# Lukeasargen/Show-Attend-and-Tell-Pytorch-Lightning

Measured on AMD Instinct MI355X. Metric: captions/sec (train step) at B=128, 256px, seq_len=22, higher is better.
Workload: dtype bf16; 1 GPU; C2: resnet50 encoder_size=7 encoder_dim=512 vocab=6400 T=22, 128 images/GPU x R=5 captions, trainable encoder, Adam, full lengths, decoder_tf=always; global_batch_images=128, parallelism=dp1, grad_bucket_dtype=fp32

## Files before the change

### show-attend-and-tell-pytorch-lightning_amd/csrc/wgrad3x3.hip

```cpp
#include <stdlib.h>

#include "gemm_bf16_common.h"
#include "profile.h"

namespace sat {

typedef int i32x4 __attribute__((ext_vector_type(4)));
typedef __attribute__((address_space(3))) void* lptr3_t;
__device__ void raw_buffer_load_lds_w(i32x4 rsrc, lptr3_t lds, int size, int voffset, int soffset, int offset, int aux) __asm("llvm.amdgcn.raw.buffer.load.lds");

namespace {
constexpr int W3_OOB = (int)0x80000000;
constexpr int W3_WAVES = 9, W3_THREADS = 64 * W3_WAVES;
constexpr int W3_MAXP = 4;
constexpr int W3_STAGES = 3;

__device__ __forceinline__ i32x4 w3_rsrc(const void* base) {
    const unsigned long long b = reinterpret_cast<unsigned long long>(base);
    i32x4 r;
    r[0] = (int)(unsigned)b; r[1] = (int)(unsigned)((b >> 32) & 0xFFFF);
    r[2] = W3_OOB; r[3] = 0x00020000;
    return r;
}

struct W3Args {
    const __bf16* dy; const __bf16* x; float* out;
    int Nimg, H, W, C, K;
    int nr;
    int units;
    int per;
    int HP;
    int Z;
};

__global__ __launch_bounds__(W3_THREADS) void wgrad3x3_kernel(W3Args a) {
    extern __shared__ __attribute__((aligned(1024))) __bf16 smem[];
    const int tid = threadIdx.x, lane = tid & 63, wave = tid >> 6;
    const int ci0 = blockIdx.x * 64, co0 = blockIdx.y * 64, bz = blockIdx.z;
    const int W = a.W, H = a.H, C = a.C, K = a.K, nr = a.nr, HW2 = W + 2;
    const int STAGE = 64 * 64 + a.HP * 64;
    const int u0 = bz * a.per, u1 = min(a.units, u0 + a.per);
    const int upi = H / nr;
    const i32x4 rA = w3_rsrc(a.dy), rX = w3_rsrc(a.x);

    const int npieces = 8 + a.HP / 8;
    int p_off[W3_MAXP]; int p_hr[W3_MAXP]; bool p_dy[W3_MAXP], p_on[W3_MAXP], p_colok[W3_MAXP]; int p_lds[W3_MAXP];
#pragma unroll
    for (int j = 0; j < W3_MAXP; ++j) {
        const int piece = j * W3_WAVES + wave;
        p_on[j] = piece < npieces; p_dy[j] = piece < 8; p_hr[j] = 0; p_colok[j] = false; p_off[j] = 0;
        const int sl = lane & 7;
        if (p_dy[j]) {
            const int krow = piece * 8 + (lane >> 3);
            const int lq = (sl >> 2) ^ ((krow >> 1) & 1);
            p_off[j] = (krow * K + co0 + (lq * 4 + (sl & 3)) * 8) * 2;
            p_lds[j] = piece * 512;
        } else {
            const int hp = (piece - 8) * 8 + (lane >> 3);
            const int hr = hp / HW2, hc = hp - hr * HW2 - 1;
            const int lq = (sl >> 2) ^ ((hp >> 1) & 1);
            p_hr[j] = hr;
            p_colok[j] = p_on[j] && hr < nr + 2 && hc >= 0 && hc < W;
            p_off[j] = ((hr * W + hc) * C + ci0 + (lq * 4 + (sl & 3)) * 8) * 2;
            p_lds[j] = 64 * 64 + (piece - 8) * 512;
        }
    }
    auto issue = [&](int buf, int u) {
        const int n = u / upi, p0 = (u - n * upi) * nr;
        const int baseA = ((n * H + p0) * W) * K * 2;
        const int baseX = ((n * H + p0 - 1) * W) * C * 2;
        __bf16* st = smem + buf * STAGE;
#pragma unroll
        for (int j = 0; j < W3_MAXP; ++j) {
            if (!p_on[j]) continue;
            if (p_dy[j]) raw_buffer_load_lds_w(rA, (lptr3_t)(st + p_lds[j]), 16, p_off[j] + baseA, 0, 0, 0);
            else {
                const int ih = p0 - 1 + p_hr[j];
                const bool ok = p_colok[j] && ih >= 0 && ih < H;
                raw_buffer_load_lds_w(rX, (lptr3_t)(st + p_lds[j]), 16, ok ? p_off[j] + baseX : W3_OOB, 0, 0, 0);
            }
        }
    };

    const int tg = lane >> 4, ti = lane & 15;
    const int t_h = tg >> 1, t_mh = tg & 1, t_q = ti >> 2, t_p = ti & 3;
    const int tap_r = wave / 3, tap_s = wave - tap_r * 3;
    int a_off[2];
#pragma unroll
    for (int i = 0; i < 2; ++i) {
        const int col = i * 32 + 16 * t_mh + 4 * t_p, kr = 8 * t_h + t_q;
        a_off[i] = kr * 64 + (((col >> 5) ^ ((kr >> 1) & 1)) << 5) + (col & 31);
    }
    int b_off[4][2][2];
#pragma unroll
    for (int ks = 0; ks < 4; ++ks)
#pragma unroll
        for (int hf = 0; hf < 2; ++hf) {
            const int k = ks * 16 + 8 * t_h + t_q + 4 * hf;
            const int pr = k / W, q = k - pr * W;
            const int hp = (pr + tap_r) * HW2 + q + tap_s;
#pragma unroll
            for (int j = 0; j < 2; ++j) {
                const int col = j * 32 + 16 * t_mh + 4 * t_p;
                b_off[ks][hf][j] = 64 * 64 + hp * 64 + (((col >> 5) ^ ((hp >> 1) & 1)) << 5) + (col & 31);
            }
        }

    f32x16 acc[2][2];
#pragma unroll
    for (int i = 0; i < 2; ++i)
#pragma unroll
        for (int j = 0; j < 2; ++j)
#pragma unroll
            for (int r = 0; r < 16; ++r) acc[i][j][r] = 0.f;

    int mine = 0;
#pragma unroll
    for (int j = 0; j < W3_MAXP; ++j) mine += p_on[j] ? 1 : 0;
    mine = __builtin_amdgcn_readfirstlane(mine);
    if (u0 < u1) {
        issue(0, u0);
        if (u0 + 1 < u1) issue(1, u0 + 1);
        int cur = 0, nxt = 2;
        for (int u = u0; u < u1; ++u) {
            if (u + 1 < u1) {
                if (mine == 4) asm volatile("s_waitcnt vmcnt(4)" ::: "memory");
                else if (mine == 3) asm volatile("s_waitcnt vmcnt(3)" ::: "memory");
                else if (mine == 2) asm volatile("s_waitcnt vmcnt(2)" ::: "memory");
                else asm volatile("s_waitcnt vmcnt(0)" ::: "memory");
            } else asm volatile("s_waitcnt vmcnt(0)" ::: "memory");
            asm volatile("s_waitcnt lgkmcnt(0)" ::: "memory");
            __builtin_amdgcn_s_barrier();
            asm volatile("" ::: "memory");
            if (u + 2 < u1) issue(nxt, u + 2);
            const __bf16* st = smem + cur * STAGE;
#pragma unroll
            for (int ks = 0; ks < 4; ++ks) {
                bf16x8 af[2], bf[2];
#pragma unroll
                for (int i = 0; i < 2; ++i) {
                    const __bf16* p = st + a_off[i] + ks * 16 * 64;
                    bf16x4 lo = __builtin_amdgcn_ds_read_tr16_b64_v4bf16((__attribute__((address_space(3))) bf16x4*)p);
                    bf16x4 hi = __builtin_amdgcn_ds_read_tr16_b64_v4bf16((__attribute__((address_space(3))) bf16x4*)(p + 4 * 64));
                    af[i] = __builtin_shufflevector(lo, hi, 0, 1, 2, 3, 4, 5, 6, 7);
                }
#pragma unroll
                for (int j = 0; j < 2; ++j) {
                    bf16x4 lo = __builtin_amdgcn_ds_read_tr16_b64_v4bf16((__attribute__((address_space(3))) bf16x4*)(st + b_off[ks][0][j]));
                    bf16x4 hi = __builtin_amdgcn_ds_read_tr16_b64_v4bf16((__attribute__((address_space(3))) bf16x4*)(st + b_off[ks][1][j]));
                    bf[j] = __builtin_shufflevector(lo, hi, 0, 1, 2, 3, 4, 5, 6, 7);
                }
#pragma unroll
                for (int i = 0; i < 2; ++i)
#pragma unroll
                    for (int j = 0; j < 2; ++j) acc[i][j] = __builtin_amdgcn_mfma_f32_32x32x16_bf16(af[i], bf[j], acc[i][j], 0, 0, 0);
            }
            cur = (cur + 1 == W3_STAGES) ? 0 : cur + 1;
            nxt = (nxt + 1 == W3_STAGES) ? 0 : nxt + 1;
        }
    }
    const int li = lane & 31, lh = lane >> 5;
    const long N9 = 9L * C;
    float* out = a.out + (a.Z > 1 ? (long)bz * K * N9 : 0L);
#pragma unroll
    for (int i = 0; i < 2; ++i)
#pragma unroll
        for (int j = 0; j < 2; ++j)
#pragma unroll
            for (int r = 0; r < 16; ++r) {
                const int row = co0 + i * 32 + (r & 3) + 8 * (r >> 2) + 4 * lh;
                const int col = ci0 + j * 32 + li;
                out[(long)row * N9 + (long)wave * C + col] = acc[i][j][r];
            }
}
}

int wgrad3x3_eligible(const ConvGeom& g) {
    if (!dev_switch(SW_WGRAD3X3)) return 0;
    if (g.R != 3 || g.S != 3 || g.stride != 1 || g.pad != 1 || (g.sw && g.sw != 1)) return 0;
    if (g.C % 64 || g.K % 64) return 0;
    if (g.H != g.P || g.W != g.Q) return 0;
    if (!(g.W == 8 || g.W == 16 || g.W == 32 || g.W == 64)) return 0;
    if (g.H % (64 / g.W)) return 0;
    if ((long)g.N * g.H * g.W * (g.C > g.K ? g.C : g.K) >= (1L << 30)) return 0;
    return 1;
}

int launch_wgrad3x3(const void* dy, const void* x, float* dw, const ConvGeom& g, float* slab, long slab_elems, hipStream_t st) {
    W3Args a;
    a.dy = reinterpret_cast<const __bf16*>(dy); a.x = reinterpret_cast<const __bf16*>(x);
    a.Nimg = g.N; a.H = g.H; a.W = g.W; a.C = g.C; a.K = g.K;
    a.nr = 64 / g.W; a.units = g.N * (g.H / a.nr);
    a.HP = ((a.nr + 2) * (g.W + 2) + 7) / 8 * 8;
    SAT_REQUIRE(8 + a.HP / 8 <= W3_WAVES * W3_MAXP, "wgrad3x3: %d LDS-DMA pieces per k-tile", 8 + a.HP / 8);
    const long tiles = (long)(g.C / 64) * (g.K / 64), out_elems = (long)g.K * 9 * g.C;
    static const int target = getenv("SAT_W3_TARGET") ? atoi(getenv("SAT_W3_TARGET")) : 256;
    long z = target / tiles; if (z < 1) z = 1;
    if (z > a.units / 8) z = a.units / 8 > 0 ? a.units / 8 : 1;
    while (z > 1 && (!slab || z * out_elems > slab_elems)) --z;
    a.per = (int)cdiv(a.units, z); a.Z = (int)cdiv(a.units, a.per);
    a.out = a.Z > 1 ? slab : dw;
    const size_t lds = W3_STAGES * (size_t)(64 * 64 + a.HP * 64) * sizeof(__bf16);
    static bool attr_set = false;
    if (!attr_set) {
        SAT_CHECK_HIP(hipFuncSetAttribute(reinterpret_cast<const void*>(&wgrad3x3_kernel), hipFuncAttributeMaxDynamicSharedMemorySize, 128 * 1024));
        attr_set = true;
    }
    {
        char pname[128];
        if (profile_enabled()) {
            static const bool shapes = getenv("SAT_PROFILE_SHAPES") != nullptr;
            if (shapes) snprintf(pname, sizeof pname, "gemm_wgrad3x3 M%d N%d K%d z%d", g.K, 9 * g.C, g.N * g.H * g.W, a.Z);
            else snprintf(pname, sizeof pname, "gemm_wgrad3x3");
        }
        ProfScope prof(pname, 2.0 * g.K * 9.0 * g.C * g.N * g.H * g.W, 2.0 * g.N * g.H * g.W * ((double)g.C + g.K) + 4.0 * out_elems, st);
        hipLaunchKernelGGL(wgrad3x3_kernel, dim3(g.C / 64, g.K / 64, a.Z), dim3(W3_THREADS), lds, st, a);
        SAT_TRY(launch_ok("wgrad3x3_kernel"));
        if (a.Z > 1) {
            BArgs k{};
            k.M = g.K; k.N = 9 * g.C; k.C = dw; k.ldc = 9 * g.C; k.slab = slab; k.nsplit = a.Z; k.wide_store = 1; k.wide_slab = 1; k.epi = EPI_NONE;
            SAT_TRY(launch_splitk_reduce<float>(k, st));
        }
    }
    return SAT_OK;
}

}
```

Measured before the change: 32510 captions/s.

## Restructure 3x3 wgrad kernel with row-ring input reuse and deeper pipeline

Rewrites the 3x3 weight-gradient kernel to keep input rows in an LDS ring buffer, so consecutive row units reuse the overlapping halo rows and load only the new rows. Waves go from 9 to 12, each owning one filter row tap and a 32x32 quadrant with three accumulators. The k-tile pipeline is deeper, with loads issued between k-steps and waits computed from outstanding counts. The kernel is templated on width, uses inline-asm buffer-to-LDS loads, and adds optional timestamp instrumentation. In exchange it needs more LDS (up to 160KB) and more complex ring bookkeeping.

New measurement: 32730 captions/s, median of 6. No clear change (+0.7%).

```diff
diff --git a/show-attend-and-tell-pytorch-lightning_amd/csrc/wgrad3x3.hip b/show-attend-and-tell-pytorch-lightning_amd/csrc/wgrad3x3.hip
--- a/show-attend-and-tell-pytorch-lightning_amd/csrc/wgrad3x3.hip
+++ b/show-attend-and-tell-pytorch-lightning_amd/csrc/wgrad3x3.hip
@@ -1,3 +1,4 @@
+#include <stdio.h>
 #include <stdlib.h>
 
 #include "gemm_bf16_common.h"
@@ -7,13 +8,19 @@
 
 typedef int i32x4 __attribute__((ext_vector_type(4)));
 typedef __attribute__((address_space(3))) void* lptr3_t;
+#ifdef SAT_DEV_TILES
 __device__ void raw_buffer_load_lds_w(i32x4 rsrc, lptr3_t lds, int size, int voffset, int soffset, int offset, int aux) __asm("llvm.amdgcn.raw.buffer.load.lds");
+#endif
 
 namespace {
 constexpr int W3_OOB = (int)0x80000000;
-constexpr int W3_WAVES = 9, W3_THREADS = 64 * W3_WAVES;
-constexpr int W3_MAXP = 4;
-constexpr int W3_STAGES = 3;
+constexpr int W3_WAVES = 12, W3_THREADS = 64 * W3_WAVES;
+constexpr int W3_LOADERS = W3_WAVES;
+constexpr int W3_MAXP = 3;
+constexpr int W3_GROUP = 2;
+constexpr int W3_MAXD = 5;
+constexpr int W3_MIND = 2 * W3_GROUP - 1;
+constexpr int W3_LDS = 160 * 1024;
 
 __device__ __forceinline__ i32x4 w3_rsrc(const void* base) {
     const unsigned long long b = reinterpret_cast<unsigned long long>(base);
@@ -23,156 +30,280 @@
     return r;
 }
 
+template <bool CDMA>
+__device__ __forceinline__ void w3_glds16(i32x4 rsrc, unsigned lds, int voffset) {
+#ifdef SAT_DEV_TILES
+    if constexpr (CDMA) { raw_buffer_load_lds_w(rsrc, (lptr3_t)(size_t)lds, 16, voffset, 0, 0, 0); return; }
+#endif
+    unsigned keep;
+    asm volatile("s_mov_b32 %0, m0\n\ts_mov_b32 m0, %2\n\ts_nop 0\n\tbuffer_load_dwordx4 %1, %3, 0 offen lds\n\ts_mov_b32 m0, %0"
+                 : "=&s"(keep) : "v"(voffset), "s"(lds), "s"(rsrc) : "memory");
+}
+
+#define W3_VMCNT(n) case n: asm volatile("s_waitcnt vmcnt(" #n ")" ::: "memory"); break;
+__device__ __forceinline__ void w3_wait_vmcnt(int n) {
+    switch (n) {
+        W3_VMCNT(0) W3_VMCNT(1) W3_VMCNT(2) W3_VMCNT(3) W3_VMCNT(4) W3_VMCNT(5) W3_VMCNT(6) W3_VMCNT(7) W3_VMCNT(8) W3_VMCNT(9)
+        W3_VMCNT(10) W3_VMCNT(11) W3_VMCNT(12) W3_VMCNT(13) W3_VMCNT(14) W3_VMCNT(15) W3_VMCNT(16) W3_VMCNT(17) W3_VMCNT(18)
+        W3_VMCNT(19) W3_VMCNT(20) W3_VMCNT(21) W3_VMCNT(22) W3_VMCNT(23)
+        default: asm volatile("s_waitcnt vmcnt(24)" ::: "memory"); break;
+    }
+}
+#undef W3_VMCNT
+static_assert(W3_MAXD * W3_MAXP <= 24, "w3_wait_vmcnt: immediates");
+
 struct W3Args {
     const __bf16* dy; const __bf16* x; float* out;
-    int Nimg, H, W, C, K;
-    int nr;
+    unsigned long long* stamps;
+    int Nimg, H, C, K;
     int units;
     int per;
-    int HP;
     int Z;
+    int D;
+    int NS;
 };
 
+constexpr int W3_SEGS = 7;
+#define W3_STAMP(t)                                                                              \
+    do {                                                                                         \
+        __builtin_amdgcn_sched_barrier(0);                                                       \
+        asm volatile("s_memtime %0\n\ts_waitcnt lgkmcnt(0)" : "=s"(t) :: "memory");              \
+        __builtin_amdgcn_sched_barrier(0);                                                       \
+    } while (0)
+
+template <int W, bool STAMP, bool CDMA>
 __global__ __launch_bounds__(W3_THREADS) void wgrad3x3_kernel(W3Args a) {
+    constexpr int NR = 64 / W;
+    constexpr int RS = (W + 2 + 7) / 8 * 8;
+    constexpr int PPR = RS / 8;
+    constexpr int ROW = RS * 64;
+    constexpr int NPF = 8 + (NR + 2) * PPR, NPC = 8 + NR * PPR;
+    static_assert(NPF <= W3_LOADERS * W3_MAXP, "wgrad3x3: LDS-DMA pieces per k-tile");
     extern __shared__ __attribute__((aligned(1024))) __bf16 smem[];
-    const int tid = threadIdx.x, lane = tid & 63, wave = tid >> 6;
+    const int tid = threadIdx.x, lane = tid & 63, wave = __builtin_amdgcn_readfirstlane(tid >> 6);
     const int ci0 = blockIdx.x * 64, co0 = blockIdx.y * 64, bz = blockIdx.z;
-    const int W = a.W, H = a.H, C = a.C, K = a.K, nr = a.nr, HW2 = W + 2;
-    const int STAGE = 64 * 64 + a.HP * 64;
+    const int H = a.H, C = a.C, K = a.K, D = a.D, NS = a.NS;
+    __bf16* const xring = smem + (D + 1) * 64 * 64;
+    const unsigned lds_dy = (unsigned)(size_t)(lptr3_t)smem, lds_x = lds_dy + (D + 1) * 64 * 64 * 2;
     const int u0 = bz * a.per, u1 = min(a.units, u0 + a.per);
-    const int upi = H / nr;
+    const int upi = H / NR;
     const i32x4 rA = w3_rsrc(a.dy), rX = w3_rsrc(a.x);
 
-    const int npieces = 8 + a.HP / 8;
-    int p_off[W3_MAXP]; int p_hr[W3_MAXP]; bool p_dy[W3_MAXP], p_on[W3_MAXP], p_colok[W3_MAXP]; int p_lds[W3_MAXP];
+    int p_off[W3_MAXP], p_ri[W3_MAXP], p_lds[W3_MAXP]; bool p_colok[W3_MAXP];
+    int cntF = 0, cntC = 0;
+    const int piece0 = wave;
 #pragma unroll
     for (int j = 0; j < W3_MAXP; ++j) {
-        const int piece = j * W3_WAVES + wave;
-        p_on[j] = piece < npieces; p_dy[j] = piece < 8; p_hr[j] = 0; p_colok[j] = false; p_off[j] = 0;
+        const int piece = j * W3_LOADERS + piece0;
+        cntF += piece < NPF ? 1 : 0; cntC += piece < NPC ? 1 : 0;
+        p_ri[j] = 0; p_colok[j] = false;
         const int sl = lane & 7;
-        if (p_dy[j]) {
+        if (piece < 8) {
             const int krow = piece * 8 + (lane >> 3);
             const int lq = (sl >> 2) ^ ((krow >> 1) & 1);
             p_off[j] = (krow * K + co0 + (lq * 4 + (sl & 3)) * 8) * 2;
-            p_lds[j] = piece * 512;
+            p_lds[j] = piece * 1024;
         } else {
-            const int hp = (piece - 8) * 8 + (lane >> 3);
-            const int hr = hp / HW2, hc = hp - hr * HW2 - 1;
-            const int lq = (sl >> 2) ^ ((hp >> 1) & 1);
-            p_hr[j] = hr;
-            p_colok[j] = p_on[j] && hr < nr + 2 && hc >= 0 && hc < W;
-            p_off[j] = ((hr * W + hc) * C + ci0 + (lq * 4 + (sl & 3)) * 8) * 2;
-            p_lds[j] = 64 * 64 + (piece - 8) * 512;
-        }
-    }
-    auto issue = [&](int buf, int u) {
-        const int n = u / upi, p0 = (u - n * upi) * nr;
-        const int baseA = ((n * H + p0) * W) * K * 2;
-        const int baseX = ((n * H + p0 - 1) * W) * C * 2;
-        __bf16* st = smem + buf * STAGE;
-#pragma unroll
-        for (int j = 0; j < W3_MAXP; ++j) {
-            if (!p_on[j]) continue;
-            if (p_dy[j]) raw_buffer_load_lds_w(rA, (lptr3_t)(st + p_lds[j]), 16, p_off[j] + baseA, 0, 0, 0);
-            else {
-                const int ih = p0 - 1 + p_hr[j];
-                const bool ok = p_colok[j] && ih >= 0 && ih < H;
-                raw_buffer_load_lds_w(rX, (lptr3_t)(st + p_lds[j]), 16, ok ? p_off[j] + baseX : W3_OOB, 0, 0, 0);
-            }
-        }
+            const int xp = piece - 8, ri = xp / PPR, seg = xp - ri * PPR;
+            const int pos = seg * 8 + (lane >> 3), hc = pos - 1;
+            const int lq = (sl >> 2) ^ ((pos >> 1) & 1);
+            p_ri[j] = ri;
+            p_colok[j] = hc >= 0 && hc < W;
+            p_off[j] = ((ri * W + hc) * C + ci0 + (lq * 4 + (sl & 3)) * 8) * 2;
+            p_lds[j] = seg * 1024;
+        }
+    }
+    int it = u0, i_n = u0 / upi, i_t = u0 - i_n * upi, i_slot = 0, i_dy = 0;
+    int i_ih0 = 0, i_np = 0, i_baseA = 0, i_baseX = 0, i_cnt = 0;
+    bool i_first = false;
+    auto issue_begin = [&]() {
+        const int p0 = i_t * NR;
+        i_first = it == u0 || i_t == 0;
+        i_ih0 = i_first ? p0 - 1 : p0 + 1; i_np = i_first ? NPF : NPC; i_cnt = i_first ? cntF : cntC;
+        i_baseA = ((i_n * H + p0) * W) * K * 2;
+        i_baseX = ((i_n * H + i_ih0) * W) * C * 2;
+    };
+    auto issue_piece = [&](int j) {
+        const int piece = j * W3_LOADERS + piece0;
+        if (piece >= i_np) return;
+        if (piece < 8) w3_glds16<CDMA>(rA, lds_dy + i_dy * 64 * 64 * 2 + p_lds[j], p_off[j] + i_baseA);
+        else {
+            const int ih = i_ih0 + p_ri[j];
+            int slot = i_slot + p_ri[j]; slot = slot >= NS ? slot - NS : slot;
+            const bool ok = p_colok[j] && ih >= 0 && ih < H;
+            w3_glds16<CDMA>(rX, lds_x + slot * ROW * 2 + p_lds[j], ok ? p_off[j] + i_baseX : W3_OOB);
+        }
+    };
+    auto issue_end = [&]() -> int {
+        i_slot += i_first ? NR + 2 : NR; i_slot = i_slot >= NS ? i_slot - NS : i_slot;
+        i_dy = i_dy == D ? 0 : i_dy + 1;
+        if (++i_t == upi) { i_t = 0; ++i_n; }
+        ++it;
+        return i_cnt;
+    };
+    auto issue = [&]() -> int {
+        issue_begin();
+#pragma unroll
+        for (int j = 0; j < W3_MAXP; ++j) issue_piece(j);
+        return issue_end();
     };
 
     const int tg = lane >> 4, ti = lane & 15;
     const int t_h = tg >> 1, t_mh = tg & 1, t_q = ti >> 2, t_p = ti & 3;
-    const int tap_r = wave / 3, tap_s = wave - tap_r * 3;
-    int a_off[2];
-#pragma unroll
-    for (int i = 0; i < 2; ++i) {
-        const int col = i * 32 + 16 * t_mh + 4 * t_p, kr = 8 * t_h + t_q;
-        a_off[i] = kr * 64 + (((col >> 5) ^ ((kr >> 1) & 1)) << 5) + (col & 31);
-    }
-    int b_off[4][2][2];
-#pragma unroll
-    for (int ks = 0; ks < 4; ++ks)
-#pragma unroll
-        for (int hf = 0; hf < 2; ++hf) {
-            const int k = ks * 16 + 8 * t_h + t_q + 4 * hf;
-            const int pr = k / W, q = k - pr * W;
-            const int hp = (pr + tap_r) * HW2 + q + tap_s;
-#pragma unroll
-            for (int j = 0; j < 2; ++j) {
-                const int col = j * 32 + 16 * t_mh + 4 * t_p;
-                b_off[ks][hf][j] = 64 * 64 + hp * 64 + (((col >> 5) ^ ((hp >> 1) & 1)) << 5) + (col & 31);
+    const int tap_r = wave >> 2, w_fh = (wave >> 1) & 1, w_ch = wave & 1;
+    int a_off;
+    {
+        const int col = w_fh * 32 + 16 * t_mh + 4 * t_p, kr = 8 * t_h + t_q;
+        a_off = kr * 64 + (((col >> 5) ^ ((kr >> 1) & 1)) << 5) + (col & 31);
+    }
+    const int b_prl = W == 8 ? t_h : 0;
+    int b_fix[3];
+#pragma unroll
+    for (int s = 0; s < 3; ++s) {
+        const int pos = 8 * t_h + t_q - b_prl * W + s;
+        const int col = w_ch * 32 + 16 * t_mh + 4 * t_p;
+        b_fix[s] = pos * 64 + (((col >> 5) ^ ((pos >> 1) & 1)) << 5) + (col & 31);
+    }
+
+    f32x16 acc[3];
+#pragma unroll
+    for (int s = 0; s < 3; ++s)
+#pragma unroll
+        for (int r = 0; r < 16; ++r) acc[s][r] = 0.f;
+
+    unsigned long long s_seg[W3_SEGS] = {0, 0, 0, 0, 0, 0, 0};
+    if (u0 < u1) {
+        int outst = 0;
+        for (int d = 0; d < D + 1 - W3_GROUP && it < u1; ++d) outst += issue();
+        int c_dy = 0, c_win = 0, c_t = u0 - (u0 / upi) * upi;
+        bool c_first = true;
+        for (int u = u0; u < u1; u += W3_GROUP) {
+            const int g = min(W3_GROUP, u1 - u);
+            unsigned long long t0 = 0, t1 = 0, t2 = 0, t3 = 0, ts = 0, tk[4] = {0, 0, 0, 0};
+            if constexpr (STAMP) W3_STAMP(t0);
+            {
+                bool f = c_first; int t = c_t;
+                for (int gi = 0; gi < g; ++gi) {
+                    outst -= f ? cntF : cntC;
+                    if (++t == upi) t = 0;
+                    f = t == 0;
+                }
             }
-        }
-
-    f32x16 acc[2][2];
-#pragma unroll
-    for (int i = 0; i < 2; ++i)
-#pragma unroll
-        for (int j = 0; j < 2; ++j)
-#pragma unroll
-            for (int r = 0; r < 16; ++r) acc[i][j][r] = 0.f;
-
-    int mine = 0;
-#pragma unroll
-    for (int j = 0; j < W3_MAXP; ++j) mine += p_on[j] ? 1 : 0;
-    mine = __builtin_amdgcn_readfirstlane(mine);
-    if (u0 < u1) {
-        issue(0, u0);
-        if (u0 + 1 < u1) issue(1, u0 + 1);
-        int cur = 0, nxt = 2;
-        for (int u = u0; u < u1; ++u) {
-            if (u + 1 < u1) {
-                if (mine == 4) asm volatile("s_waitcnt vmcnt(4)" ::: "memory");
-                else if (mine == 3) asm volatile("s_waitcnt vmcnt(3)" ::: "memory");
-                else if (mine == 2) asm volatile("s_waitcnt vmcnt(2)" ::: "memory");
-                else asm volatile("s_waitcnt vmcnt(0)" ::: "memory");
-            } else asm volatile("s_waitcnt vmcnt(0)" ::: "memory");
+            w3_wait_vmcnt(outst);
+            if constexpr (STAMP) W3_STAMP(t1);
             asm volatile("s_waitcnt lgkmcnt(0)" ::: "memory");
             __builtin_amdgcn_s_barrier();
             asm volatile("" ::: "memory");
-            if (u + 2 < u1) issue(nxt, u + 2);
-            const __bf16* st = smem + cur * STAGE;
-#pragma unroll
-            for (int ks = 0; ks < 4; ++ks) {
-                bf16x8 af[2], bf[2];
-#pragma unroll
-                for (int i = 0; i < 2; ++i) {
-                    const __bf16* p = st + a_off[i] + ks * 16 * 64;
-                    bf16x4 lo = __builtin_amdgcn_ds_read_tr16_b64_v4bf16((__attribute__((address_space(3))) bf16x4*)p);
-                    bf16x4 hi = __builtin_amdgcn_ds_read_tr16_b64_v4bf16((__attribute__((address_space(3))) bf16x4*)(p + 4 * 64));
-                    af[i] = __builtin_shufflevector(lo, hi, 0, 1, 2, 3, 4, 5, 6, 7);
+            if constexpr (STAMP) { W3_STAMP(t2); s_seg[0] += t1 - t0; s_seg[1] += t2 - t1; }
+#pragma unroll
+            for (int gi = 0; gi < W3_GROUP; ++gi) {
+                if (gi >= g) break;
+                if constexpr (STAMP) W3_STAMP(ts);
+                const bool more = it < u1;
+                if (more) issue_begin();
+                if constexpr (STAMP) W3_STAMP(t3);
+                const __bf16* st = smem + c_dy * 64 * 64;
+#pragma unroll
+                for (int ks = 0; ks < 4; ++ks) {
+                    const int prs = (ks * 16) / W, qs = (ks * 16) % W;
+                    int row = c_win + tap_r + prs + b_prl; row = row >= NS ? row - NS : row;
+                    const __bf16* rb = xring + row * ROW + qs * 64;
+                    bf16x8 af, bf[3];
+                    {
+                        const __bf16* p = st + a_off + ks * 16 * 64;
+                        bf16x4 lo = __builtin_amdgcn_ds_read_tr16_b64_v4bf16((__attribute__((address_space(3))) bf16x4*)p);
+                        bf16x4 hi = __builtin_amdgcn_ds_read_tr16_b64_v4bf16((__attribute__((address_space(3))) bf16x4*)(p + 4 * 64));
+                        af = __builtin_shufflevector(lo, hi, 0, 1, 2, 3, 4, 5, 6, 7);
+                    }
+#pragma unroll
+                    for (int s = 0; s < 3; ++s) {
+                        bf16x4 lo = __builtin_amdgcn_ds_read_tr16_b64_v4bf16((__attribute__((address_space(3))) bf16x4*)(rb + b_fix[s]));
+                        bf16x4 hi = __builtin_amdgcn_ds_read_tr16_b64_v4bf16((__attribute__((address_space(3))) bf16x4*)(rb + b_fix[s] + 4 * 64));
+                        bf[s] = __builtin_shufflevector(lo, hi, 0, 1, 2, 3, 4, 5, 6, 7);
+                    }
+#pragma unroll
+                    for (int s = 0; s < 3; ++s) acc[s] = __builtin_amdgcn_mfma_f32_32x32x16_bf16(af, bf[s], acc[s], 0, 0, 0);
+                    if (more && ks < W3_MAXP) issue_piece(ks);
+                    if constexpr (STAMP) W3_STAMP(tk[ks]);
                 }
-#pragma unroll
-                for (int j = 0; j < 2; ++j) {
-                    bf16x4 lo = __builtin_amdgcn_ds_read_tr16_b64_v4bf16((__attribute__((address_space(3))) bf16x4*)(st + b_off[ks][0][j]));
-                    bf16x4 hi = __builtin_amdgcn_ds_read_tr16_b64_v4bf16((__attribute__((address_space(3))) bf16x4*)(st + b_off[ks][1][j]));
-                    bf[j] = __builtin_shufflevector(lo, hi, 0, 1, 2, 3, 4, 5, 6, 7);
+                if (more) outst += issue_end();
+                if constexpr (STAMP) {
+                    s_seg[2] += t3 - ts;
+                    s_seg[3] += tk[0] - t3; s_seg[4] += tk[1] - tk[0]; s_seg[5] += tk[2] - tk[1]; s_seg[6] += tk[3] - tk[2];
                 }
-#pragma unroll
-                for (int i = 0; i < 2; ++i)
-#pragma unroll
-                    for (int j = 0; j < 2; ++j) acc[i][j] = __builtin_amdgcn_mfma_f32_32x32x16_bf16(af[i], bf[j], acc[i][j], 0, 0, 0);
+                if (++c_t == upi) c_t = 0;
+                c_first = c_t == 0;
+                c_win += c_first ? NR + 2 : NR; c_win = c_win >= NS ? c_win - NS : c_win;
+                c_dy = c_dy == D ? 0 : c_dy + 1;
             }
-            cur = (cur + 1 == W3_STAGES) ? 0 : cur + 1;
-            nxt = (nxt + 1 == W3_STAGES) ? 0 : nxt + 1;
+        }
+    }
+    if constexpr (STAMP) {
+        if (lane == 0 && a.stamps) {
+            const long wg = ((long)bz * gridDim.y + blockIdx.y) * gridDim.x + blockIdx.x;
+#pragma unroll
+            for (int s = 0; s < W3_SEGS; ++s) a.stamps[(wg * W3_WAVES + wave) * W3_SEGS + s] = s_seg[s];
         }
     }
     const int li = lane & 31, lh = lane >> 5;
     const long N9 = 9L * C;
     float* out = a.out + (a.Z > 1 ? (long)bz * K * N9 : 0L);
 #pragma unroll
-    for (int i = 0; i < 2; ++i)
-#pragma unroll
-        for (int j = 0; j < 2; ++j)
-#pragma unroll
-            for (int r = 0; r < 16; ++r) {
-                const int row = co0 + i * 32 + (r & 3) + 8 * (r >> 2) + 4 * lh;
-                const int col = ci0 + j * 32 + li;
-                out[(long)row * N9 + (long)wave * C + col] = acc[i][j][r];
-            }
-}
+    for (int s = 0; s < 3; ++s)
+#pragma unroll
+        for (int r = 0; r < 16; ++r) {
+            const int row = co0 + w_fh * 32 + (r & 3) + 8 * (r >> 2) + 4 * lh;
+            const int col = ci0 + w_ch * 32 + li;
+            out[(long)row * N9 + (long)(tap_r * 3 + s) * C + col] = acc[s][r];
+        }
+}
+#undef W3_STAMP
+
+template <int W, bool STAMP, bool CDMA>
+int w3_launch(const W3Args& a, dim3 grid, size_t lds, hipStream_t st) {
+    static bool attr_set = false;
+    if (!attr_set) {
+        SAT_CHECK_HIP(hipFuncSetAttribute(reinterpret_cast<const void*>(&wgrad3x3_kernel<W, STAMP, CDMA>), hipFuncAttributeMaxDynamicSharedMemorySize, W3_LDS));
+        attr_set = true;
+    }
+    hipLaunchKernelGGL((wgrad3x3_kernel<W, STAMP, CDMA>), grid, dim3(W3_THREADS), lds, st, a);
+    return SAT_OK;
+}
+
+template <bool STAMP, bool CDMA>
+int w3_launch_w(int W, const W3Args& a, dim3 grid, size_t lds, hipStream_t st) {
+    if (W == 64) return w3_launch<64, STAMP, CDMA>(a, grid, lds, st);
+    if (W == 32) return w3_launch<32, STAMP, CDMA>(a, grid, lds, st);
+    if (W == 16) return w3_launch<16, STAMP, CDMA>(a, grid, lds, st);
+    return w3_launch<8, STAMP, CDMA>(a, grid, lds, st);
+}
+
+inline int w3_ring_rows(int D, int nr, int upi) { return (D + 1) * nr + 2 + 2 * ((D + upi - 1) / upi); }
+inline size_t w3_lds_bytes(int D, int NS, int W) { return ((size_t)(D + 1) * 64 * 64 + (size_t)NS * ((W + 2 + 7) / 8 * 8) * 64) * sizeof(__bf16); }
+
+#ifdef SAT_DEV_TILES
+int w3_stamped_launch(int W, W3Args a, dim3 grid, size_t lds, const ConvGeom& g, hipStream_t st) {
+    const size_t n = (size_t)grid.x * grid.y * grid.z * W3_WAVES * W3_SEGS;
+    const bool cdma = getenv("SAT_W3_CDMA") != nullptr;
+    unsigned long long* dev = nullptr;
+    SAT_CHECK_HIP(hipMalloc(&dev, n * sizeof *dev));
+    (void)hipMemsetAsync(dev, 0, n * sizeof *dev, st);
+    a.stamps = dev;
+    if (cdma) SAT_TRY((w3_launch_w<true, true>(W, a, grid, lds, st)));
+    else SAT_TRY((w3_launch_w<true, false>(W, a, grid, lds, st)));
+    unsigned long long* host = (unsigned long long*)malloc(n * sizeof *host);
+    (void)hipStreamSynchronize(st);
+    (void)hipMemcpy(host, dev, n * sizeof *host, hipMemcpyDeviceToHost);
+    double seg[W3_SEGS] = {0, 0, 0, 0, 0, 0, 0}, all = 0;
+    for (size_t i = 0; i < n; ++i) { seg[i % W3_SEGS] += (double)host[i]; all += (double)host[i]; }
+    const double tiles = (double)a.per * (n / W3_SEGS);
+    fprintf(stderr, "w3_stamps %s N%d H%d W%d C%d K%d D%d NS%d z%d per%d: wait %.1f%% barrier %.1f%% set-up %.1f%% k-steps %.1f%% %.1f%% %.1f%% %.1f%%  (%.0f s_memtime ticks per k-tile and wave)\n",
+            cdma ? "counted-dma" : "asm-dma", g.N, g.H, g.W, g.C, g.K, a.D, a.NS, a.Z, a.per, 100 * seg[0] / all, 100 * seg[1] / all, 100 * seg[2] / all,
+            100 * seg[3] / all, 100 * seg[4] / all, 100 * seg[5] / all, 100 * seg[6] / all, all / tiles);
+    free(host); (void)hipFree(dev);
+    return SAT_OK;
+}
+#endif
 }
 
 int wgrad3x3_eligible(const ConvGeom& g) {
@@ -188,11 +319,10 @@
 
 int launch_wgrad3x3(const void* dy, const void* x, float* dw, const ConvGeom& g, float* slab, long slab_elems, hipStream_t st) {
     W3Args a;
-    a.dy = reinterpret_cast<const __bf16*>(dy); a.x = reinterpret_cast<const __bf16*>(x);
-    a.Nimg = g.N; a.H = g.H; a.W = g.W; a.C = g.C; a.K = g.K;
-    a.nr = 64 / g.W; a.units = g.N * (g.H / a.nr);
-    a.HP = ((a.nr + 2) * (g.W + 2) + 7) / 8 * 8;
-    SAT_REQUIRE(8 + a.HP / 8 <= W3_WAVES * W3_MAXP, "wgrad3x3: %d LDS-DMA pieces per k-tile", 8 + a.HP / 8);
+    a.dy = reinterpret_cast<const __bf16*>(dy); a.x = reinterpret_cast<const __bf16*>(x); a.stamps = nullptr;
+    a.Nimg = g.N; a.H = g.H; a.C = g.C; a.K = g.K;
+    const int nr = 64 / g.W, upi = g.H / nr;
+    a.units = g.N * upi;
     const long tiles = (long)(g.C / 64) * (g.K / 64), out_elems = (long)g.K * 9 * g.C;
     static const int target = getenv("SAT_W3_TARGET") ? atoi(getenv("SAT_W3_TARGET")) : 256;
     long z = target / tiles; if (z < 1) z = 1;
@@ -200,12 +330,17 @@
     while (z > 1 && (!slab || z * out_elems > slab_elems)) --z;
     a.per = (int)cdiv(a.units, z); a.Z = (int)cdiv(a.units, a.per);
     a.out = a.Z > 1 ? slab : dw;
-    const size_t lds = W3_STAGES * (size_t)(64 * 64 + a.HP * 64) * sizeof(__bf16);
-    static bool attr_set = false;
-    if (!attr_set) {
-        SAT_CHECK_HIP(hipFuncSetAttribute(reinterpret_cast<const void*>(&wgrad3x3_kernel), hipFuncAttributeMaxDynamicSharedMemorySize, 128 * 1024));
-        attr_set = true;
-    }
+    int D = W3_MIND;
+#ifdef SAT_DEV_TILES
+    if (getenv("SAT_W3_DEPTH")) D = atoi(getenv("SAT_W3_DEPTH"));
+    if (D > W3_MAXD) D = W3_MAXD;
+#endif
+    if (D < W3_MIND) D = W3_MIND;
+    while (D > W3_MIND && w3_lds_bytes(D, w3_ring_rows(D, nr, upi), g.W) > (size_t)W3_LDS) --D;
+    a.D = D; a.NS = w3_ring_rows(D, nr, upi);
+    const size_t lds = w3_lds_bytes(a.D, a.NS, g.W);
+    SAT_REQUIRE(lds <= (size_t)W3_LDS, "wgrad3x3: %zu bytes of LDS", lds);
+    const dim3 grid(g.C / 64, g.K / 64, a.Z);
     {
         char pname[128];
         if (profile_enabled()) {
@@ -214,7 +349,11 @@
             else snprintf(pname, sizeof pname, "gemm_wgrad3x3");
         }
         ProfScope prof(pname, 2.0 * g.K * 9.0 * g.C * g.N * g.H * g.W, 2.0 * g.N * g.H * g.W * ((double)g.C + g.K) + 4.0 * out_elems, st);
-        hipLaunchKernelGGL(wgrad3x3_kernel, dim3(g.C / 64, g.K / 64, a.Z), dim3(W3_THREADS), lds, st, a);
+#ifdef SAT_DEV_TILES
+        if (getenv("SAT_W3_STAMPS")) SAT_TRY(w3_stamped_launch(g.W, a, grid, lds, g, st));
+        else
+#endif
+        SAT_TRY((w3_launch_w<false, false>(g.W, a, grid, lds, st)));
         SAT_TRY(launch_ok("wgrad3x3_kernel"));
         if (a.Z > 1) {
             BArgs k{};
```
